# Mirko-Nava/BayesianNeuralNetworks

Measured on AMD Instinct MI355X. Metric: MC-samples/sec (node), 784-1200-1200-10 BayesianLinear MLP, batch 512, higher is better.
Workload: dtype bf16

## Files before the change

bayesianneuralnetworks_amd/_lib.py:

```python
import ctypes
import os

import torch

_HERE = os.path.dirname(os.path.abspath(__file__))
LIB_PATH = os.environ.get("BNN_HIP_LIB") or os.path.join(_HERE, "libbnn_hip.so")

F32, BF16, BF16X3 = 0, 1, 2
COMPUTE_F32, COMPUTE_BF16 = 0, 1
FLAG_RELU = 1
FLAG_X_BF16 = 2
E_ALIGN, E_UNSUPPORTED, E_DEVICE = -4, -6, -7
FLAG_Y_BF16 = 4


class BnnHipError(RuntimeError):
    pass


ABI_VERSION = 2


class Rng(ctypes.Structure):
    _fields_ = [("seed", ctypes.c_uint64),
# ... 39 lines not shown

_p = ctypes.c_void_p
_i64 = ctypes.c_int64
_int = ctypes.c_int
_f = ctypes.c_float
_rngp = ctypes.POINTER(Rng)

SIGNATURES = {
    "bnn_abi_version": (_int, []),
    "bnn_arch": (ctypes.c_char_p, []),
    "bnn_last_error": (ctypes.c_char_p, []),
    "bnn_launch_count": (ctypes.c_uint64, []),
    "bnn_set_workspace": (_int, [_int, _p, _i64]),
    "bnn_check_device": (_int, [_int, _p]),
    "bnn_sample_affine_eps": (_int, [_p, _p, _p, _p, _i64, _int, _p]),
    "bnn_sample_affine_philox": (_int, [_p, _p, _p, _i64, _int, _i64, _int, _rngp, _p]),
    "bnn_eps_philox": (_int, [_p, _i64, _int, _i64, _rngp, _p]),
    "bnn_sigma": (_int, [_p, _p, _i64, _p]),
    "bnn_sample_affine_bwd": (_int, [_p, _i64, _p, _p, _i64, _rngp, _i64, _int, _p, _p, _int, _p]),
    "bnn_rng_advance": (_int, [_p, ctypes.c_uint32, _p]),
    "bnn_prune_score": (_int, [_p, _p, _p, _i64, _p]),
    "bnn_kl_workspace_bytes": (_i64, [_int]),
    "bnn_kl_forward": (_int, [ctypes.POINTER(KlTensor), _int, _f, _p, _p, _p]),
    "bnn_kl_forward_partial": (_int, [ctypes.POINTER(KlTensor), _int, _p, _p]),
    "bnn_kl_backward": (_int, [ctypes.POINTER(KlTensor), _int, _f, _p, ctypes.POINTER(_p),
                               ctypes.POINTER(_p), _int, _p]),
    "bnn_linear_forward_sampled": (_int, [_p, _i64, _i64, _p, _p, _p, _p, _p, _i64, _i64, _i64, _i64,
                                          _i64, _int, _rngp, _rngp, _int, _int, _p]),
    "bnn_linear_forward_sampled_kl": (_int, [_p, _i64, _i64, _p, _p, _p, _p, _p, _i64, _i64, _i64, _i64,
                                             _i64, _int, _rngp, _rngp, _int, _int, ctypes.POINTER(KlTensor), _int, _p, _p]),
    "bnn_draw_multi": (_int, [ctypes.POINTER(DrawTensor), _int, _int, ctypes.POINTER(KlTensor), _int, _p, _p]),
    "bnn_dense_forward": (_int, [_p, _i64, _i64, _p, _i64, _i64, _p, _i64, _p, _i64, _i64, _i64, _i64, _i64, _int, _int, _p]),
    "bnn_dense_head_parts": (_int, [_i64, _i64, _int]),
    "bnn_dense_forward_head": (_int, [_p, _i64, _i64, _p, _i64, _i64, _p, _i64, _p, _i64, _i64, _p, _i64, _i64,
                                      _p, _i64, _i64, _i64, _int, _int, _p]),
    "bnn_dense_forward_x3_head": (_int, [_p, _i64, _i64, _i64, _p, _i64, _i64, _i64, _p, _i64, _p, _i64, _i64, _i64,
                                         _p, _i64, _i64, _p, _i64, _i64, _i64, _int, _int, _p]),
    "bnn_dense_forward_x3": (_int, [_p, _i64, _i64, _i64, _p, _i64, _i64, _i64, _p, _i64, _p, _i64, _i64, _i64,
                                    _i64, _i64, _i64, _int, _int, _p]),
    "bnn_split_bf16x3": (_int, [_p, _i64, _i64, _i64, _p, _i64, _i64, _p]),
    "bnn_transpose_bf16": (_int, [_p, _i64, _i64, _p, _i64, _i64, _i64, _i64, _int, _p]),
    "bnn_conv2d_dense_forward_x3": (_int, [_p, _i64, _p, _i64, _i64, _i64, _p, _i64, _p, _i64, ctypes.POINTER(Conv2dShape), _int, _int, _p]),
    "bnn_conv2d_dense_forward": (_int, [_p, _i64, _p, _i64, _i64, _p, _i64, _p, _i64, ctypes.POINTER(Conv2dShape), _int, _int, _p]),
    "bnn_conv2d_flipout_forward": (_int, [_p, _p, _i64, _p, _p, _p, ctypes.POINTER(Conv2dShape), _int, _p]),
    "bnn_conv2d_flipout_forward_x3": (_int, [_p, _p, _i64, _i64, _p, _p, _p, ctypes.POINTER(Conv2dShape), _int, _p]),
    "bnn_linear_forward": (_int, [_p, _i64, _i64, _p, _i64, _p, _i64, _p, _i64, _i64, _i64, _i64, _i64,
                                  _int, _int, _int, _p]),
    "bnn_linear_backward_input_sampled": (_int, [_p, _i64, _i64, _p, _p, _p, _i64, _i64, _i64, _i64, _i64, _int,
                                                 _rngp, _int, _int, _p]),
    "bnn_linear_backward_input": (_int, [_p, _i64, _i64, _p, _i64, _p, _i64, _i64, _i64, _i64, _i64, _int, _int, _p]),
    "bnn_linear_backward_weight_sampled": (_int, [_p, _i64, _i64, _p, _i64, _i64, _p, _p, _p, _p, _p, _p, _i64, _i64,
                                                  _i64, _int, _rngp, _rngp, ctypes.POINTER(KlFuse), _int, _int, _int, _p]),
    "bnn_linear_backward_narrow_sampled": (_int, [_p, _i64, _i64, _p, _i64, _i64, _p, _p, _p, _i64, _i64, _p, _p, _p, _p, _p,
                                                  _i64, _i64, _i64, _int, _rngp, _rngp, ctypes.POINTER(KlFuse), _int, _int, _p]),
    "bnn_linear_backward_weight": (_int, [_p, _i64, _i64, _p, _i64, _i64, _p, _i64, _i64, _i64, _i64, _int, _int,
                                          _int, _int, _p]),
    "bnn_colsum": (_int, [_p, _i64, _i64, _p, _i64, _i64, _int, _int, _p]),
    "bnn_relu_backward": (_int, [_p, _p, _p, _i64, _int, _p]),
    "bnn_adam_step": (_int, [ctypes.POINTER(AdamTensor), _int, _f, _f, _f, _f, _f, _p, _p]),
    "bnn_adam_step_advance": (_int, [ctypes.POINTER(AdamTensor), _int, _f, _f, _f, _f, _f, _p, _p, ctypes.c_uint32, _p]),
    "bnn_xent_workspace_bytes": (_i64, [_i64]),
    "bnn_softmax_xent": (_int, [_p, _p, _i64, _int, _p, _p, _p, _p]),
    "bnn_conv2d_im2col": (_int, [_p, _i64, ctypes.POINTER(Conv2dShape), _int, _p, _int, _p]),
    "bnn_conv2d_col2im": (_int, [_p, ctypes.POINTER(Conv2dShape), _int, _int, _p, _p]),
    "bnn_nchw_to_rows": (_int, [_p, _i64, _int, _int, _p, _int, _p]),
    "bnn_conv2d_workspace_bytes": (_i64, [ctypes.POINTER(Conv2dShape), _int, _int]),
# ... 117 lines not shown
```

bayesianneuralnetworks_amd/csrc/bnn_dense.hip:

```cpp
#include <cstdlib>
#include <type_traits>

#include "bnn_device.hpp"
#include "bnn_dma.hpp"
#include "bnn_kl_body.hpp"

namespace bnn {

typedef float f32x4 __attribute__((ext_vector_type(4)));
typedef __bf16 bf16x8 __attribute__((ext_vector_type(8)));

constexpr int kDrawMaxTensors = 8;
constexpr int kDrawSpreadBelow = 4096;

struct DrawTensorDev {
    const float *mu;
    const float *rho;
    void *out;
    int64_t out_sample_stride;
    int32_t rows, cols, ld;
    int32_t bf16;
    int32_t kind;
    int32_t perm_taps;
    int32_t first_item;
// ... 357 lines not shown
        }
    }
}

struct DenseParams {
    const uint16_t *A;
    int64_t a_sample_stride;
    int64_t lda;
    const uint16_t *W;
    int64_t w_sample_stride;
    int64_t ldw;
    const float *bias;
    int64_t bias_sample_stride;
    void *Y;
    int64_t y_sample_stride;
    int64_t ldy;
    int32_t M, N, K, S;
    int32_t ntm, ntn;
    int32_t flags;
    int32_t x3;
    int64_t a_plane_stride, w_plane_stride, y_plane_stride;
    const uint16_t *Wh;
    int64_t wh_sample_stride, ldwh;
    const float *bias_h;
    int64_t bias_h_sample_stride;
    float *P;
    int32_t Nh;
    int64_t wh_plane_stride;
};

constexpr int kDenseLoaderPrio = 1 << 21;
constexpr int kDenseNoXcdMap = 1 << 20;

__device__ __forceinline__ void dma_piece(const void *base, uint32_t voff, uint32_t lds)
{
    uint32_t keep;
    asm volatile("s_mov_b32 %0, m0\n\ts_mov_b32 m0, %3\n\ts_nop 0\n\tglobal_load_lds_dwordx4 %1, %2\n\ts_mov_b32 m0, %0"
                 : "=&s"(keep) : "v"(voff), "s"(base), "s"(lds) : "memory");
}

template <int TM, int TN, int NWM, int NWN, int ST, int YM, bool RELU, int DIAG = 0>
__global__ __launch_bounds__(512) void k_dense_bf16(const DenseParams p)
{
    constexpr int NWV = 4;
    constexpr bool INTERLEAVE = true;
    constexpr int MPR = DIAG == 3 ? 1 : DIAG == 4 ? 2 : TN >= 8 ? 2 : 1;
    static_assert(NWM * NWN == NWV, "four consumer waves");
    constexpr int WM = 16 * TM, WN = 16 * TN, BM = NWM * WM, BN = NWN * WN;
    constexpr int A_TOTAL = BM / 8;
    constexpr int B_TOTAL = BN / 8;
    static_assert(A_TOTAL % NWV == 0, "A pieces divide evenly over the loaders");
    constexpr int A_PIECES = A_TOTAL / NWV;
    constexpr int B_BASE = B_TOTAL / NWV, B_EXTRA = B_TOTAL % NWV;
    constexpr int A_STAGE = BM * 128;
    constexpr int B_STAGE = BN * 128;
    constexpr int STAGE = A_STAGE + B_STAGE;
    constexpr bool YBF = YM != 0;
    constexpr int ESZ = YBF ? 2 : 4;
    constexpr int EPI_BYTES = ST * STAGE / NWV;
    constexpr int EPI_A = (EPI_BYTES / (16 * (WN * ESZ + 16))) < TM ? (EPI_BYTES / (16 * (WN * ESZ + 16))) : TM;
    static_assert(EPI_A >= 1, "a quarter of the ring must hold at least 16 output rows (epilogue staging)");
    __shared__ __attribute__((aligned(16))) char lds[ST * STAGE];

    const int per_s = p.ntm * p.ntn;
    int s, t;
    {
        const int L = (int)blockIdx.x;
        if (p.flags & kDenseNoXcdMap) {
            s = L / per_s;
            t = L % per_s;
        } else if (p.S % 8 == 0) {
            const int idx = L >> 3;
            s = (L & 7) + 8 * (idx / per_s);
            t = idx % per_s;
        } else {
            const int total = per_s * p.S, x = L & 7;
            const int u = x * (total >> 3) + (x < (total & 7) ? x : (total & 7)) + (L >> 3);
            s = u / per_s;
            t = u % per_s;
        }
    }
    int mt, panel;
    if (per_s > 32 && !(p.flags & kDenseNoXcdMap)) {
        constexpr int GM = 4;
        const int grp = t / (GM * p.ntn), first = grp * GM;
        const int gm = p.ntm - first < GM ? p.ntm - first : GM;
        const int v = t - grp * (GM * p.ntn);
        mt = first + v % gm;
        panel = v / gm;
    } else {
        mt = t / p.ntn;
        panel = t % p.ntn;
    }
    const int m0 = mt * BM, n0 = panel * BN;
    const int tid = threadIdx.x, lane = tid & 63;
    const int wave = __builtin_amdgcn_readfirstlane(tid >> 6);
    const int nk = (p.K + 63) / 64 * (p.x3 ? 6 : 1);

    if (wave >= NWV) {
        const int lw = wave - NWV;
        if (p.flags & kDenseLoaderPrio) __builtin_amdgcn_s_setprio(2);
        const uint32_t ring = __builtin_amdgcn_readfirstlane(lds_addr_of(lds));
        const int prow = lane >> 3;
        const int schunk = (lane & 7) ^ prow;
        const char *a_base = reinterpret_cast<const char *>(p.A + (int64_t)s * p.a_sample_stride);
        const char *w_base = reinterpret_cast<const char *>(p.W + (int64_t)s * p.w_sample_stride);
        uint32_t a_off[A_PIECES], b_off[B_BASE + 1];
        uint32_t a_dst[A_PIECES], b_dst[B_BASE + 1];
#pragma unroll
        for (int j = 0; j < A_PIECES; ++j) {
            const int r0 = (lw + NWV * j) * 8;
            int m = m0 + r0 + prow;
            m = m < p.M ? m : p.M - 1;
            a_off[j] = (uint32_t)((int64_t)m * p.lda * 2);
            a_dst[j] = (uint32_t)((r0 / WM) * (ST * WM * 128) + (r0 % WM) * 128);
        }
#pragma unroll
        for (int j = 0; j < B_BASE + 1; ++j) {
            const int r0 = (lw + NWV * j) * 8;
            int n = n0 + r0 + prow;
            n = n < p.N ? n : p.N - 1;
            b_off[j] = (uint32_t)((int64_t)n * p.ldw * 2) + 16u * (uint32_t)schunk;
            b_dst[j] = (uint32_t)(ST * A_STAGE + (r0 / WN) * (ST * WN * 128) + (r0 % WN) * 128);
        }
        const uint32_t a_colmax = (uint32_t)(p.K * 2 - 16);
        auto run = [&](auto nbp_c) {
            constexpr int NBP = decltype(nbp_c)::value;
            constexpr int P = A_PIECES + NBP;
            auto issue = [&](int kt) {
                if constexpr (DIAG == 2 || DIAG == 5 || DIAG == 8 || DIAG == 9) return;
                const int stage = kt % ST;
                int kb = kt;
                const char *ab = a_base, *wb = w_base;
                if (p.x3) {
                    const int nkb = (p.K + 63) >> 6;
                    int pr = 5;
                    if (kt < 5 * nkb) { kb = kt / 5; pr = kt - 5 * kb; } else kb = kt - 5 * nkb;
                    ab += ((0x001102 >> (4 * pr)) & 3) * (p.a_plane_stride * 2);
                    wb += ((0x010120 >> (4 * pr)) & 3) * (p.w_plane_stride * 2);
                }
                const uint32_t colA0 = (uint32_t)(kb * 128 + 16 * schunk);
                const uint32_t colA = colA0 < a_colmax ? colA0 : a_colmax;
                const uint32_t colB = (uint32_t)(kb * 128);
                const uint32_t sa = ring + (uint32_t)(stage * (WM * 128)), sb = ring + (uint32_t)(stage * (WN * 128));
#pragma unroll
                for (int j = 0; j < A_PIECES; ++j)
                    dma_piece(ab, a_off[j] + colA, sa + a_dst[j]);
#pragma unroll
                for (int j = 0; j < NBP; ++j)
                    dma_piece(wb, b_off[j] + colB, sb + b_dst[j]);
            };
#pragma unroll
            for (int i = 0; i < ST - 1; ++i)
                if (i < nk) issue(i);
            for (int kt = 0; kt < nk; ++kt) {
                const int ahead = nk - 1 - kt < ST - 2 ? nk - 1 - kt : ST - 2;
                if (ST >= 4 && ahead == 2) asm volatile("s_waitcnt vmcnt(%0)" :: "n"(2 * P) : "memory");
                else if (ahead >= 1) asm volatile("s_waitcnt vmcnt(%0)" :: "n"(P) : "memory");
                else asm volatile("s_waitcnt vmcnt(0)" ::: "memory");
                if constexpr (DIAG != 5 && DIAG != 9) __builtin_amdgcn_s_barrier();
                if (kt + ST - 1 < nk) issue(kt + ST - 1);
            }
            __builtin_amdgcn_s_barrier();
        };
        if (lw < B_EXTRA) run(std::integral_constant<int, B_BASE + 1>{});
        else run(std::integral_constant<int, B_BASE>{});
        return;
    }

    static_assert(ST == 3 || ST == 4, "ring depth");
    uint64_t stamp[5] = {0, 0, 0, 0, 0};
    if constexpr (DIAG >= 6) stamp[0] = __builtin_amdgcn_s_memrealtime();
    const int fi = lane & 15, fq = lane >> 4;
    const int wm = wave / NWN, wn = wave % NWN;
    const char *a_rows = lds + wm * (ST * WM * 128);
    const char *b_rows = lds + ST * A_STAGE + wn * (ST * WN * 128);
    __builtin_amdgcn_s_setprio(1);
    f32x4 acc[TM][TN];
#pragma unroll
    for (int a = 0; a < TM; ++a)
#pragma unroll
        for (int b = 0; b < TN; ++b) acc[a][b] = f32x4{0.f, 0.f, 0.f, 0.f};
    const int fbase0 = fi * 128 + (((0 + fq) ^ (fi & 7)) << 4);
    const int fbase1 = fi * 128 + (((4 + fq) ^ (fi & 7)) << 4);
    uint4 fa[2][TM], fb[2][TN];
    auto rd = [&](auto buf_c, uint32_t stage, auto h_c) {
        constexpr int buf = decltype(buf_c)::value, h = decltype(h_c)::value;
        if constexpr (DIAG == 1 || DIAG == 7) return;
        const char *As = a_rows + (stage * (uint32_t)(WM * 128) + (uint32_t)(h ? fbase1 : fbase0));
        const char *Bs = b_rows + (stage * (uint32_t)(WN * 128) + (uint32_t)(h ? fbase1 : fbase0));
#pragma unroll
        for (int b = 0; b < TN; ++b) fb[buf][b] = *reinterpret_cast<const uint4 *>(Bs + b * 2048);
#pragma unroll
        for (int a = 0; a < TM; ++a) fa[buf][a] = *reinterpret_cast<const uint4 *>(As + a * 2048);
    };
    auto mm = [&](auto buf_c) {
        constexpr int buf = decltype(buf_c)::value;
        if constexpr (DIAG == 1 || DIAG == 7) return;
#pragma unroll
        for (int a = 0; a < TM; ++a)
#pragma unroll
            for (int b = 0; b < TN; ++b)
                acc[a][b] = __builtin_amdgcn_mfma_f32_16x16x32_bf16(__builtin_bit_cast(bf16x8, fb[buf][b]),
                                                                    __builtin_bit_cast(bf16x8, fa[buf][a]), acc[a][b], 0, 0, 0);
    };
    using I0 = std::integral_constant<int, 0>;
    using I1 = std::integral_constant<int, 1>;
    auto interleave = [&]() {
        if constexpr ((DIAG == 0 || (DIAG >= 3 && DIAG != 7)) && INTERLEAVE) {
            constexpr int NI = (TM * TN) / MPR < TM + TN ? (TM * TN) / MPR : TM + TN;
#pragma unroll
            for (int i = 0; i < NI; ++i) {
                __builtin_amdgcn_sched_group_barrier(0x008, MPR, 0);
                __builtin_amdgcn_sched_group_barrier(0x100, 1, 0);
            }
            if constexpr (TM + TN > NI) __builtin_amdgcn_sched_group_barrier(0x100, TM + TN - NI, 0);
            if constexpr (TM * TN > MPR * NI) __builtin_amdgcn_sched_group_barrier(0x008, TM * TN - MPR * NI, 0);
        }
    };
    auto first_half = [&](uint32_t stage) {
        rd(I1{}, stage, I1{});
        if constexpr (!INTERLEAVE) __builtin_amdgcn_sched_barrier(0);
        mm(I0{});
        interleave();
        __builtin_amdgcn_sched_barrier(0);
    };
    auto second_half = [&](uint32_t next) {
        asm volatile("s_waitcnt lgkmcnt(0)" ::: "memory");
        if constexpr (DIAG != 5 && DIAG != 9) __builtin_amdgcn_s_barrier();
        asm volatile("" ::: "memory");
        rd(I0{}, next, I0{});
        if constexpr (!INTERLEAVE) __builtin_amdgcn_sched_barrier(0);
        mm(I1{});
        interleave();
        __builtin_amdgcn_sched_barrier(0);
    };
    const float *bias = p.bias ? p.bias + (int64_t)s * p.bias_sample_stride : nullptr;
    const int mw = m0 + wm * WM, nw = n0 + wn * WN;
    constexpr bool BIAS_PRE = TM * TN <= 20;
    float bv[TN][4];
    auto load_bias = [&]() {
#pragma unroll
        for (int b = 0; b < TN; ++b)
#pragma unroll
            for (int r = 0; r < 4; ++r) {
                const int n = nw + b * 16 + fq * 4 + r;
                bv[b][r] = (bias && n < p.N) ? bias[n] : 0.f;
            }
    };
    if constexpr (BIAS_PRE) load_bias();
    if (DIAG == 0 && (nw >= p.N || mw >= p.M)) {
        for (int kt = 0; kt < nk + 1; ++kt) __builtin_amdgcn_s_barrier();
        if constexpr (YM == 3) {
            float *P = p.P + ((int64_t)(panel * NWN + wn) * p.S + s) * (int64_t)p.M * p.Nh;
            for (int i = lane; i < WM * p.Nh; i += 64) {
                const int m = mw + i / p.Nh;
                if (m < p.M) P[(int64_t)m * p.Nh + (i % p.Nh)] = 0.f;
            }
        }
        return;
    }
    if constexpr (DIAG != 5 && DIAG != 9) __builtin_amdgcn_s_barrier();
    asm volatile("" ::: "memory");
    if constexpr (DIAG >= 6) stamp[1] = __builtin_amdgcn_s_memrealtime();
    rd(I0{}, 0u, I0{});
    uint32_t stage = 0;
    for (int kt = 0; kt + 1 < nk; ++kt) {
        const uint32_t next = stage + 1 == (uint32_t)ST ? 0u : stage + 1;
        first_half(stage);
        second_half(next);
        stage = next;
    }
    first_half(stage);
    mm(I1{});
    __builtin_amdgcn_sched_barrier(0);
    __builtin_amdgcn_s_setprio(0);
    asm volatile("s_waitcnt lgkmcnt(0)" ::: "memory");
    __builtin_amdgcn_s_barrier();
    asm volatile("" ::: "memory");
    if constexpr (DIAG >= 6) stamp[2] = __builtin_amdgcn_s_memrealtime();
    auto leave_stamps = [&]() {
        if constexpr (DIAG >= 6) {
            stamp[3] = __builtin_amdgcn_s_memrealtime();
            asm volatile("s_waitcnt vmcnt(0)" ::: "memory");
            stamp[4] = __builtin_amdgcn_s_memrealtime();
            if (wave == 0 && lane == 0 && p.P) {
                uint64_t *q = reinterpret_cast<uint64_t *>(p.P) + (int64_t)blockIdx.x * 5;
                for (int i = 0; i < 5; ++i) q[i] = stamp[i];
            }
        }
    };

    if constexpr (!BIAS_PRE) load_bias();
    const int64_t ybase = (int64_t)s * p.y_sample_stride * ESZ;
    auto vals = [&](int a, int b, float (&v)[4]) {
#pragma unroll
        for (int r = 0; r < 4; ++r) {
            v[r] = acc[a][b][r] + bv[b][r];
            if (RELU) v[r] = fmaxf(v[r], 0.f);
        }
    };
    if constexpr (YM == 3) {
        constexpr bool X3_HEAD_FITS = 3 * WM * (WN * 2 + 16) <= EPI_BYTES;
        if constexpr (X3_HEAD_FITS) if (p.x3) {
            constexpr int pitch = WN * 2 + 16;
            char *T = lds + wave * EPI_BYTES;
#pragma unroll
            for (int a = 0; a < TM; ++a)
#pragma unroll
                for (int b = 0; b < TN; ++b) {
                    float v[4];
                    vals(a, b, v);
                    uint32_t h0, m0, l0, h1, m1, l1;
                    split_bf16x3(v[0], v[1], h0, m0, l0);
                    split_bf16x3(v[2], v[3], h1, m1, l1);
                    char *q = T + (a * 16 + fi) * pitch + (b * 16 + fq * 4) * 2;
                    *reinterpret_cast<uint2 *>(q) = make_uint2(h0, h1);
                    *reinterpret_cast<uint2 *>(q + WM * pitch) = make_uint2(m0, m1);
                    *reinterpret_cast<uint2 *>(q + 2 * WM * pitch) = make_uint2(l0, l1);
                }
            __builtin_amdgcn_fence(__ATOMIC_RELEASE, "workgroup");
            __builtin_amdgcn_wave_barrier();
            const int Nh = p.Nh;
            const int hrow = fi < Nh ? fi : Nh - 1;
            const uint16_t *wh = p.Wh + (int64_t)s * p.wh_sample_stride + (int64_t)hrow * p.ldwh;
            f32x4 hacc[TM], hsm[TM];
#pragma unroll
            for (int a = 0; a < TM; ++a) { hacc[a] = f32x4{0.f, 0.f, 0.f, 0.f}; hsm[a] = hacc[a]; }
            constexpr int NC = (WN + 31) / 32;
#pragma unroll
            for (int c = 0; c < NC; ++c) {
                const int kcol = 32 * c + 8 * fq;
                const int n = nw + kcol;
                const bool okb = kcol < WN && fi < Nh && n + 8 <= (int)p.ldwh;
                uint4 bf[3];
#pragma unroll
                for (int pl = 0; pl < 3; ++pl)
                    bf[pl] = okb ? *reinterpret_cast<const uint4 *>(wh + pl * p.wh_plane_stride + n) : make_uint4(0u, 0u, 0u, 0u);
#pragma unroll
                for (int a = 0; a < TM; ++a) {
                    uint4 af[3];
#pragma unroll
                    for (int pl = 0; pl < 3; ++pl)
                        af[pl] = kcol < WN ? *reinterpret_cast<const uint4 *>(T + pl * WM * pitch + (a * 16 + fi) * pitch + kcol * 2) : make_uint4(0u, 0u, 0u, 0u);
                    auto mf = [&](f32x4 c4, int pa, int pw) {
                        return __builtin_amdgcn_mfma_f32_16x16x32_bf16(__builtin_bit_cast(bf16x8, af[pa]), __builtin_bit_cast(bf16x8, bf[pw]), c4, 0, 0, 0);
                    };
                    hsm[a] = mf(mf(mf(mf(mf(hsm[a], 2, 0), 0, 2), 1, 1), 1, 0), 0, 1);
                    hacc[a] = mf(hacc[a], 0, 0);
                }
            }
            const int part = panel * NWN + wn;
            float hb = 0.f;
            if (part == 0 && p.bias_h && fi < Nh) hb = p.bias_h[(int64_t)s * p.bias_h_sample_stride + fi];
            float *P = p.P + ((int64_t)part * p.S + s) * (int64_t)p.M * Nh;
#pragma unroll
            for (int a = 0; a < TM; ++a)
#pragma unroll
                for (int r = 0; r < 4; ++r) {
                    const int m = mw + a * 16 + fq * 4 + r;
                    if (m < p.M && fi < Nh) P[(int64_t)m * Nh + fi] = (hacc[a][r] + hsm[a][r]) + hb;
                }
            return;
        }
        constexpr int pitch = WN * 2 + 16;
        static_assert(WM * pitch <= EPI_BYTES, "the wave's quarter of the ring holds its bf16 tile");
        char *T = lds + wave * EPI_BYTES;
#pragma unroll
        for (int a = 0; a < TM; ++a)
#pragma unroll
            for (int b = 0; b < TN; ++b) {
                float v[4];
                vals(a, b, v);
                *reinterpret_cast<uint2 *>(T + (a * 16 + fi) * pitch + (b * 16 + fq * 4) * 2) = make_uint2(pack_bf16x2(v[0], v[1]), pack_bf16x2(v[2], v[3]));
            }
        __builtin_amdgcn_fence(__ATOMIC_RELEASE, "workgroup");
        __builtin_amdgcn_wave_barrier();
        const int Nh = p.Nh;
        const int hrow = fi < Nh ? fi : Nh - 1;
        const uint16_t *wh = p.Wh + (int64_t)s * p.wh_sample_stride + (int64_t)hrow * p.ldwh;
        f32x4 hacc[TM];
#pragma unroll
        for (int a = 0; a < TM; ++a) hacc[a] = f32x4{0.f, 0.f, 0.f, 0.f};
        constexpr int NC = (WN + 31) / 32;
#pragma unroll
        for (int c = 0; c < NC; ++c) {
            const int kcol = 32 * c + 8 * fq;
            const int n = nw + kcol;
            uint4 bf = make_uint4(0u, 0u, 0u, 0u);
            if (kcol < WN && fi < Nh && n + 8 <= (int)p.ldwh) bf = *reinterpret_cast<const uint4 *>(wh + n);
#pragma unroll
            for (int a = 0; a < TM; ++a) {
                uint4 af = make_uint4(0u, 0u, 0u, 0u);
                if (kcol < WN) af = *reinterpret_cast<const uint4 *>(T + (a * 16 + fi) * pitch + kcol * 2);
                hacc[a] = __builtin_amdgcn_mfma_f32_16x16x32_bf16(__builtin_bit_cast(bf16x8, af), __builtin_bit_cast(bf16x8, bf), hacc[a], 0, 0, 0);
            }
        }
        const int part = panel * NWN + wn;
        float hb = 0.f;
        if (part == 0 && p.bias_h && fi < Nh) hb = p.bias_h[(int64_t)s * p.bias_h_sample_stride + fi];
        float *P = p.P + ((int64_t)part * p.S + s) * (int64_t)p.M * Nh;
#pragma unroll
        for (int a = 0; a < TM; ++a)
#pragma unroll
            for (int r = 0; r < 4; ++r) {
                const int m = mw + a * 16 + fq * 4 + r;
                if (m < p.M && fi < Nh) P[(int64_t)m * Nh + fi] = hacc[a][r] + hb;
            }
        return;
    }
    auto plane_of = [&](float v, int pl) -> uint16_t {
        const uint16_t h = f2bf(v);
        if (pl == 0) return h;
        const float r = v - __uint_as_float((uint32_t)h << 16);
        const uint16_t m = f2bf(r);
        if (pl == 1) return m;
        return f2bf(r - __uint_as_float((uint32_t)m << 16));
    };
    constexpr int NP = YM == 2 ? 3 : 1;
    const bool wide = nw + WN <= p.N && mw + WM <= p.M && (p.ldy * ESZ) % 16 == 0 && (nw * ESZ) % 16 == 0 &&
                      ((reinterpret_cast<uintptr_t>(p.Y) + ybase) & 15u) == 0 && (NP == 1 || (p.y_plane_stride * ESZ) % 16 == 0);
    if (wide) {
        char *T = lds + wave * EPI_BYTES;
        constexpr int row_bytes = WN * ESZ;
        constexpr int pitch = row_bytes + 16;
        constexpr int cpr = row_bytes / 16;
#pragma unroll
        for (int pl = 0; pl < NP; ++pl) {
            char *Y8 = reinterpret_cast<char *>(p.Y) + ybase + ((int64_t)pl * p.y_plane_stride + (int64_t)mw * p.ldy + nw) * ESZ;
#pragma unroll
            for (int a0 = 0; a0 < TM; a0 += EPI_A) {
#pragma unroll
                for (int b = 0; b < TN; ++b)
#pragma unroll
                    for (int a = a0; a < a0 + EPI_A && a < TM; ++a) {
                        float v[4];
                        vals(a, b, v);
                        char *q = T + ((a - a0) * 16 + fi) * pitch + (b * 16 + fq * 4) * ESZ;
                        if (YM == 2)
                            *reinterpret_cast<uint2 *>(q) = make_uint2((uint32_t)plane_of(v[0], pl) | ((uint32_t)plane_of(v[1], pl) << 16),
                                                                       (uint32_t)plane_of(v[2], pl) | ((uint32_t)plane_of(v[3], pl) << 16));
                        else if (YM == 1) *reinterpret_cast<uint2 *>(q) = make_uint2(pack_bf16x2(v[0], v[1]), pack_bf16x2(v[2], v[3]));
                        else *reinterpret_cast<float4 *>(q) = make_float4(v[0], v[1], v[2], v[3]);
                    }
                __builtin_amdgcn_fence(__ATOMIC_RELEASE, "workgroup");
                __builtin_amdgcn_wave_barrier();
                const int nrows = (TM - a0 < EPI_A ? TM - a0 : EPI_A) * 16;
                for (int c = lane; c < nrows * cpr; c += 64) {
                    const int row = c / cpr, cc = c - row * cpr;
                    *reinterpret_cast<uint4 *>(Y8 + (int64_t)(a0 * 16 + row) * p.ldy * ESZ + cc * 16) =
                        *reinterpret_cast<const uint4 *>(T + row * pitch + cc * 16);
                }
                __builtin_amdgcn_fence(__ATOMIC_RELEASE, "workgroup");
                __builtin_amdgcn_wave_barrier();
            }
        }
        leave_stamps();
        return;
    }
    float *Yf = reinterpret_cast<float *>(p.Y) + (int64_t)s * p.y_sample_stride;
    uint16_t *Yh = reinterpret_cast<uint16_t *>(p.Y) + (int64_t)s * p.y_sample_stride;
#pragma unroll
    for (int a = 0; a < TM; ++a) {
        const int m = mw + a * 16 + fi;
        if (m >= p.M) continue;
#pragma unroll
        for (int b = 0; b < TN; ++b) {
            float v[4];
            vals(a, b, v);
#pragma unroll
            for (int r = 0; r < 4; ++r) {
                const int n = nw + b * 16 + fq * 4 + r;
                if (n >= p.N) continue;
                if (YM == 2) {
#pragma unroll
                    for (int pl = 0; pl < 3; ++pl) Yh[(int64_t)pl * p.y_plane_stride + (int64_t)m * p.ldy + n] = plane_of(v[r], pl);
                } else if (YM == 1) Yh[(int64_t)m * p.ldy + n] = f2bf(v[r]);
                else Yf[(int64_t)m * p.ldy + n] = v[r];
            }
        }
    }
}

constexpr int kHeadMaxSteps = 16;

__global__ __launch_bounds__(256) void k_head_bf16(const DenseParams p)
{
    __shared__ float red[4][16][17];
    const int ntm = p.ntm;
    const int s = (int)blockIdx.x / ntm, mt = (int)blockIdx.x % ntm;
    const int tid = threadIdx.x, lane = tid & 63, wave = tid >> 6;
    const int fi = lane & 15, fq = lane >> 4;
    const int nk = (p.K + 31) / 32;
    const int per = (nk + 3) / 4;
    const int k0 = wave * per, k1 = (k0 + per < nk) ? k0 + per : nk;
    int m = mt * 16 + fi;
    m = m < p.M ? m : p.M - 1;
    int n = fi < p.N ? fi : p.N - 1;
    const uint16_t *arow = p.A + (int64_t)s * p.a_sample_stride + (int64_t)m * p.lda;
    const uint16_t *wrow = p.W + (int64_t)s * p.w_sample_stride + (int64_t)n * p.ldw;
    uint4 af[kHeadMaxSteps], bfr[kHeadMaxSteps];
    const int kmax = p.K - 8;
    f32x4 acc = f32x4{0.f, 0.f, 0.f, 0.f};
    const int npass = p.x3 ? 6 : 1;
    for (int pass = 0; pass < npass; ++pass) {
        const uint16_t *ar = arow, *wr = wrow;
        if (p.x3) {
            ar += ((0x001102 >> (4 * pass)) & 3) * p.a_plane_stride;
            wr += ((0x010120 >> (4 * pass)) & 3) * p.w_plane_stride;
        }
#pragma unroll
        for (int i = 0; i < kHeadMaxSteps; ++i) {
            const int kt = k0 + i;
            int ka = kt * 32 + 8 * fq;
// ... 591 lines not shown
                    d.kl_prior_mu = kl_tensors[j].prior_mu; d.kl_prior_sigma = kl_tensors[j].prior_sigma;
                    in_items = true;
                }
            }
            L.kl.pg_first[j] = launched;
            if (!in_items) launched += nb;
        }
        L.kl.pg_first[kl_ntensors] = launched;
        L.kl.nblocks = launched;
        grid += L.kl.nblocks;
    }
    int split = 1;
    while (split < nsamples && (int64_t)L.draw_blocks * split < 1024) split *= 2;
    if (split > nsamples) split = nsamples;
    static const int force_split = [] { const char *e = getenv("BNN_DRAW_SPLIT"); return e ? atoi(e) : 0; }();
    if (force_split >= 1 && force_split <= nsamples) split = force_split;
    static const int unroll = [] { const char *e = getenv("BNN_DRAW_UNROLL"); return e ? atoi(e) : 1; }();
    if (unroll == 2) hipLaunchKernelGGL(k_draw_multi<2>, dim3((unsigned)grid, (unsigned)split), dim3(256), 0, (hipStream_t)stream, L);
    else if (unroll == 4) hipLaunchKernelGGL(k_draw_multi<4>, dim3((unsigned)grid, (unsigned)split), dim3(256), 0, (hipStream_t)stream, L);
    else if (unroll == 8) hipLaunchKernelGGL(k_draw_multi<8>, dim3((unsigned)grid, (unsigned)split), dim3(256), 0, (hipStream_t)stream, L);
    else
    hipLaunchKernelGGL(k_draw_multi<1>, dim3((unsigned)grid, (unsigned)split), dim3(256), 0, (hipStream_t)stream, L);
    return check_launch(who);
}

int bnn_dense_forward(const void *x, int64_t x_sample_stride, int64_t ldx,
                      const void *w, int64_t w_sample_stride, int64_t ldw,
                      const float *b, int64_t b_sample_stride,
                      void *y, int64_t y_sample_stride, int64_t ldy,
                      int64_t M, int64_t N, int64_t K, int nsamples, int flags, void *stream)
{
    return dense_launch("bnn_dense_forward", x, 0, x_sample_stride, ldx, w, 0, w_sample_stride, ldw, b, b_sample_stride,
                        y, 0, y_sample_stride, ldy, M, N, K, nsamples, flags, false, stream);
}

int bnn_dense_head_parts(int64_t M, int64_t N, int nsamples)
{
    if (M < 1 || N < 17 || nsamples < 1) return 0;
    const int tile = dense_pick_tile(M, N, nsamples);
    const int bn = tile == 0 ? 80 : tile == 2 ? 128 : 160;
    const int nwn = (tile == 0 || tile == 2) ? 1 : 2;
    return (int)((N + bn - 1) / bn) * nwn;
}

int bnn_dense_forward_head(const void *x, int64_t x_sample_stride, int64_t ldx,
                           const void *w, int64_t w_sample_stride, int64_t ldw,
                           const float *b, int64_t b_sample_stride,
                           const void *w_head, int64_t wh_sample_stride, int64_t ldwh,
                           const float *b_head, int64_t bh_sample_stride, int64_t n_head,
                           float *partials, int64_t M, int64_t N, int64_t K, int nsamples, int flags, void *stream)
{
    HeadArgs h{w_head, 0, wh_sample_stride, ldwh, b_head, bh_sample_stride, partials, n_head};
    return dense_launch("bnn_dense_forward_head", x, 0, x_sample_stride, ldx, w, 0, w_sample_stride, ldw, b, b_sample_stride,
                        nullptr, 0, 0, N, M, N, K, nsamples, flags | BNN_FLAG_Y_BF16, false, stream, &h);
}

int bnn_dense_forward_x3_head(const void *x, int64_t x_plane_stride, int64_t x_sample_stride, int64_t ldx,
                              const void *w, int64_t w_plane_stride, int64_t w_sample_stride, int64_t ldw,
                              const float *b, int64_t b_sample_stride,
                              const void *w_head, int64_t wh_plane_stride, int64_t wh_sample_stride, int64_t ldwh,
                              const float *b_head, int64_t bh_sample_stride, int64_t n_head,
                              float *partials, int64_t M, int64_t N, int64_t K, int nsamples, int flags, void *stream)
{
    if (wh_plane_stride <= 0) { set_error("bnn_dense_forward_x3_head: plane stride of the head's weights"); return BNN_E_SHAPE; }
    HeadArgs h{w_head, wh_plane_stride, wh_sample_stride, ldwh, b_head, bh_sample_stride, partials, n_head};
    return dense_launch("bnn_dense_forward_x3_head", x, x_plane_stride, x_sample_stride, ldx, w, w_plane_stride, w_sample_stride, ldw,
// ... 155 lines not shown
```

include/bnn_hip.h:

```cpp
#ifndef BNN_HIP_H
#define BNN_HIP_H

#include <stdint.h>

#ifdef __cplusplus
extern "C" {
#endif

#define BNN_ABI_VERSION 2

enum {
    BNN_OK = 0,
    BNN_E_NULL = -1,
    BNN_E_SHAPE = -2,
    BNN_E_DTYPE = -3,
    BNN_E_ALIGN = -4,
    BNN_E_RANGE = -5,
    BNN_E_UNSUPPORTED = -6,
    BNN_E_DEVICE = -7
};

enum { BNN_F32 = 0, BNN_BF16 = 1,
       BNN_BF16X3 = 2  };

// ... 63 lines not shown
int bnn_linear_forward_sampled(const void *x, int64_t x_sample_stride, int64_t ldx,
                               const float *mu_w, const float *rho_w,
                               const float *mu_b, const float *rho_b,
                               void *y, int64_t y_sample_stride, int64_t ldy,
                               int64_t M, int64_t N, int64_t K, int nsamples,
                               const bnn_rng_t *rng_w, const bnn_rng_t *rng_b,
                               int compute, int flags, void *stream);
int bnn_linear_forward_sampled_kl(const void *x, int64_t x_sample_stride, int64_t ldx,
                                  const float *mu_w, const float *rho_w, const float *mu_b,
                                  const float *rho_b, void *y, int64_t y_sample_stride, int64_t ldy,
                                  int64_t M, int64_t N, int64_t K, int nsamples, const bnn_rng_t *rng_w,
                                  const bnn_rng_t *rng_b, int compute, int flags,
                                  const bnn_kl_tensor_t *tensors, int ntensors, void *kl_workspace, void *stream);
typedef struct bnn_draw_tensor {
    const float *mu;
    const float *rho;
    int64_t rows, cols;
    void *out;
    int64_t ld;
    int64_t out_sample_stride;
    int out_dtype;
    int kind;
    int taps;
    bnn_rng_t rng;
} bnn_draw_tensor_t;
int bnn_draw_multi(const bnn_draw_tensor_t *tensors, int ntensors, int nsamples,
                   const bnn_kl_tensor_t *kl_tensors, int kl_ntensors, void *kl_workspace, void *stream);
int bnn_dense_forward(const void *x, int64_t x_sample_stride, int64_t ldx,
                      const void *w, int64_t w_sample_stride, int64_t ldw,
                      const float *b, int64_t b_sample_stride,
                      void *y, int64_t y_sample_stride, int64_t ldy,
                      int64_t M, int64_t N, int64_t K, int nsamples, int flags, void *stream);
int bnn_dense_head_parts(int64_t M, int64_t N, int nsamples);
int bnn_dense_forward_head(const void *x, int64_t x_sample_stride, int64_t ldx,
                           const void *w, int64_t w_sample_stride, int64_t ldw,
                           const float *b, int64_t b_sample_stride,
                           const void *w_head, int64_t wh_sample_stride, int64_t ldwh,
                           const float *b_head, int64_t bh_sample_stride, int64_t n_head,
                           float *partials, int64_t M, int64_t N, int64_t K, int nsamples, int flags, void *stream);
int bnn_dense_forward_x3_head(const void *x, int64_t x_plane_stride, int64_t x_sample_stride, int64_t ldx,
                              const void *w, int64_t w_plane_stride, int64_t w_sample_stride, int64_t ldw,
                              const float *b, int64_t b_sample_stride,
                              const void *w_head, int64_t wh_plane_stride, int64_t wh_sample_stride, int64_t ldwh,
                              const float *b_head, int64_t bh_sample_stride, int64_t n_head,
                              float *partials, int64_t M, int64_t N, int64_t K, int nsamples, int flags, void *stream);
int bnn_dense_forward_x3(const void *x, int64_t x_plane_stride, int64_t x_sample_stride, int64_t ldx,
                         const void *w, int64_t w_plane_stride, int64_t w_sample_stride, int64_t ldw,
                         const float *b, int64_t b_sample_stride,
                         void *y, int64_t y_plane_stride, int64_t y_sample_stride, int64_t ldy,
                         int64_t M, int64_t N, int64_t K, int nsamples, int flags, void *stream);
int bnn_split_bf16x3(const float *x, int64_t rows, int64_t cols, int64_t ldx, void *out, int64_t ld_out, int64_t plane_stride,
                     void *stream);
int bnn_transpose_bf16(const void *in, int64_t in_batch_stride, int64_t ld_in, void *out, int64_t out_batch_stride, int64_t ld_out,
                       int64_t rows, int64_t cols, int batch, void *stream);

int bnn_linear_forward(const float *x, int64_t x_sample_stride, int64_t ldx,
                       const float *w, int64_t w_sample_stride,
                       const float *b, int64_t b_sample_stride,
                       float *y, int64_t y_sample_stride, int64_t ldy,
                       int64_t M, int64_t N, int64_t K, int nsamples,
                       int compute, int flags, void *stream);

int bnn_linear_backward_input_sampled(const void *gy, int64_t gy_sample_stride, int64_t ldgy,
                                      const float *mu_w, const float *rho_w,
                                      void *gx, int64_t gx_sample_stride, int64_t ldgx,
                                      int64_t M, int64_t N, int64_t K, int nsamples,
// ... 119 lines not shown
```

Before: 188,700.

## Trim dense GEMM tail-tile work and stage bias through LDS via DMA

Loader waves now compute how many B rows the tile actually covers and issue only those DMA pieces. For single-column-wave TN=8 tiles, the consumer picks a reduced TNE at runtime so partial last N tiles skip their MFMAs and LDS reads. Bias for large tiles is prefetched into an extra LDS slot by a loader wave instead of being read from global memory in the epilogue, and base pointers are forced into SGPRs. This adds template instantiations and code size, and the wide-store path now masks partial columns. A query function for the chosen tile is also exported.

```diff
diff --git a/bayesianneuralnetworks_amd/_lib.py b/bayesianneuralnetworks_amd/_lib.py
--- a/bayesianneuralnetworks_amd/_lib.py
+++ b/bayesianneuralnetworks_amd/_lib.py
@@ -95,6 +95,7 @@
     "bnn_draw_multi": (_int, [ctypes.POINTER(DrawTensor), _int, _int, ctypes.POINTER(KlTensor), _int, _p, _p]),
     "bnn_dense_forward": (_int, [_p, _i64, _i64, _p, _i64, _i64, _p, _i64, _p, _i64, _i64, _i64, _i64, _i64, _int, _int, _p]),
     "bnn_dense_head_parts": (_int, [_i64, _i64, _int]),
+    "bnn_dense_tile": (_int, [_i64, _i64, _int]),
     "bnn_dense_forward_head": (_int, [_p, _i64, _i64, _p, _i64, _i64, _p, _i64, _p, _i64, _i64, _p, _i64, _i64,
                                       _p, _i64, _i64, _i64, _int, _int, _p]),
     "bnn_dense_forward_x3_head": (_int, [_p, _i64, _i64, _i64, _p, _i64, _i64, _i64, _p, _i64, _p, _i64, _i64, _i64,
diff --git a/bayesianneuralnetworks_amd/csrc/bnn_dense.hip b/bayesianneuralnetworks_amd/csrc/bnn_dense.hip
--- a/bayesianneuralnetworks_amd/csrc/bnn_dense.hip
+++ b/bayesianneuralnetworks_amd/csrc/bnn_dense.hip
@@ -413,6 +413,13 @@
 constexpr int kDenseLoaderPrio = 1 << 21;
 constexpr int kDenseNoXcdMap = 1 << 20;
 
+__device__ __forceinline__ const char *sgpr_ptr(const void *p)
+{
+    const uint64_t v = reinterpret_cast<uint64_t>(p);
+    const uint32_t lo = __builtin_amdgcn_readfirstlane((uint32_t)v), hi = __builtin_amdgcn_readfirstlane((uint32_t)(v >> 32));
+    return reinterpret_cast<const char *>(((uint64_t)hi << 32) | lo);
+}
+
 __device__ __forceinline__ void dma_piece(const void *base, uint32_t voff, uint32_t lds)
 {
     uint32_t keep;
@@ -420,12 +427,26 @@
                  : "=&s"(keep) : "v"(voff), "s"(base), "s"(lds) : "memory");
 }
 
+__device__ __forceinline__ void dma_dword(const void *base, uint32_t voff, uint32_t lds)
+{
+    uint32_t keep;
+    asm volatile("s_mov_b32 %0, m0\n\ts_mov_b32 m0, %3\n\ts_nop 0\n\tglobal_load_lds_dword %1, %2\n\ts_mov_b32 m0, %0"
+                 : "=&s"(keep) : "v"(voff), "s"(base), "s"(lds) : "memory");
+}
+
+template <int LO, int HI, class F>
+__device__ __forceinline__ void with_count(int n, F &&f)
+{
+    if constexpr (LO >= HI) f(std::integral_constant<int, HI>{});
+    else if (n <= LO) f(std::integral_constant<int, LO>{});
+    else with_count<LO + 1, HI>(n, f);
+}
+
 template <int TM, int TN, int NWM, int NWN, int ST, int YM, bool RELU, int DIAG = 0>
 __global__ __launch_bounds__(512) void k_dense_bf16(const DenseParams p)
 {
     constexpr int NWV = 4;
     constexpr bool INTERLEAVE = true;
-    constexpr int MPR = DIAG == 3 ? 1 : DIAG == 4 ? 2 : TN >= 8 ? 2 : 1;
     static_assert(NWM * NWN == NWV, "four consumer waves");
     constexpr int WM = 16 * TM, WN = 16 * TN, BM = NWM * WM, BN = NWN * WN;
     constexpr int A_TOTAL = BM / 8;
@@ -441,7 +462,11 @@
     constexpr int EPI_BYTES = ST * STAGE / NWV;
     constexpr int EPI_A = (EPI_BYTES / (16 * (WN * ESZ + 16))) < TM ? (EPI_BYTES / (16 * (WN * ESZ + 16))) : TM;
     static_assert(EPI_A >= 1, "a quarter of the ring must hold at least 16 output rows (epilogue staging)");
-    __shared__ __attribute__((aligned(16))) char lds[ST * STAGE];
+    constexpr bool BIAS_PRE = TM * TN <= 20;
+    constexpr int BIAS_SLOT = BIAS_PRE ? 0 : BN * 4;
+    static_assert(BN % 64 == 0 || BIAS_PRE, "the bias slot is filled 64 columns at a time");
+    __shared__ __attribute__((aligned(16))) char lds[ST * STAGE + BIAS_SLOT];
+    constexpr bool TN_SPLIT = NWN == 1 && TN == 8 && (DIAG == 0 || DIAG == 6);
 
     const int per_s = p.ntm * p.ntn;
     int s, t;
@@ -477,6 +502,8 @@
     const int tid = threadIdx.x, lane = tid & 63;
     const int wave = __builtin_amdgcn_readfirstlane(tid >> 6);
     const int nk = (p.K + 63) / 64 * (p.x3 ? 6 : 1);
+    const int pcols = p.N - n0;
+    const int brows = TN_SPLIT ? (pcols < BN ? (pcols + 15) / 16 * 16 : BN) : (pcols < BN ? (pcols + WN - 1) / WN * WN : BN);
 
     if (wave >= NWV) {
         const int lw = wave - NWV;
@@ -484,8 +511,8 @@
         const uint32_t ring = __builtin_amdgcn_readfirstlane(lds_addr_of(lds));
         const int prow = lane >> 3;
         const int schunk = (lane & 7) ^ prow;
-        const char *a_base = reinterpret_cast<const char *>(p.A + (int64_t)s * p.a_sample_stride);
-        const char *w_base = reinterpret_cast<const char *>(p.W + (int64_t)s * p.w_sample_stride);
+        const char *a_base = sgpr_ptr(p.A + (int64_t)s * p.a_sample_stride);
+        const char *w_base = sgpr_ptr(p.W + (int64_t)s * p.w_sample_stride);
         uint32_t a_off[A_PIECES], b_off[B_BASE + 1];
         uint32_t a_dst[A_PIECES], b_dst[B_BASE + 1];
 #pragma unroll
@@ -505,7 +532,17 @@
             b_dst[j] = (uint32_t)(ST * A_STAGE + (r0 / WN) * (ST * WN * 128) + (r0 % WN) * 128);
         }
         const uint32_t a_colmax = (uint32_t)(p.K * 2 - 16);
-        auto run = [&](auto nbp_c) {
+        if constexpr (!BIAS_PRE) {
+            if (lw == 0 && p.bias) {
+                const char *bb = sgpr_ptr(p.bias + (int64_t)s * p.bias_sample_stride);
+#pragma unroll
+                for (int j = 0; j < BN / 64; ++j) {
+                    const int n = n0 + 64 * j + lane;
+                    dma_dword(bb, (uint32_t)(n < p.N ? n : p.N - 1) * 4u, ring + (uint32_t)(ST * STAGE + 256 * j));
+                }
+            }
+        }
+        auto run = [&](auto nbp_c) __attribute__((always_inline)) {
             constexpr int NBP = decltype(nbp_c)::value;
             constexpr int P = A_PIECES + NBP;
             auto issue = [&](int kt) {
@@ -544,8 +581,24 @@
             }
             __builtin_amdgcn_s_barrier();
         };
-        if (lw < B_EXTRA) run(std::integral_constant<int, B_BASE + 1>{});
-        else run(std::integral_constant<int, B_BASE>{});
+        const int nbp_all = lw < B_EXTRA ? B_BASE + 1 : B_BASE;
+        const int nbp_read = (brows / 8 - lw + NWV - 1) / NWV;
+        const int nbp = __builtin_amdgcn_readfirstlane(nbp_read < nbp_all ? nbp_read : nbp_all);
+        if (nbp == B_BASE + 1) run(std::integral_constant<int, B_BASE + 1>{});
+        else if (nbp == B_BASE) run(std::integral_constant<int, B_BASE>{});
+        else if constexpr (B_BASE >= 1) {
+            if (nbp == B_BASE - 1) run(std::integral_constant<int, B_BASE - 1>{});
+            else if constexpr (B_BASE >= 2) {
+                if (nbp == B_BASE - 2) run(std::integral_constant<int, B_BASE - 2>{});
+                else if constexpr (B_BASE >= 3) {
+                    if (nbp == B_BASE - 3) run(std::integral_constant<int, B_BASE - 3>{});
+                    else if constexpr (B_BASE >= 4) {
+                        if (nbp == B_BASE - 4) run(std::integral_constant<int, B_BASE - 4>{});
+                        else if constexpr (B_BASE >= 5) { if (nbp == B_BASE - 5) run(std::integral_constant<int, B_BASE - 5>{}); }
+                    }
+                }
+            }
+        }
         return;
     }
 
@@ -557,21 +610,24 @@
     const char *a_rows = lds + wm * (ST * WM * 128);
     const char *b_rows = lds + ST * A_STAGE + wn * (ST * WN * 128);
     __builtin_amdgcn_s_setprio(1);
-    f32x4 acc[TM][TN];
+    auto consume = [&](auto tne_c) __attribute__((always_inline)) {
+    constexpr int TNE = decltype(tne_c)::value, WNE = 16 * TNE;
+    constexpr int MPRE = DIAG == 3 ? 1 : DIAG == 4 ? 2 : TNE >= 8 ? 2 : 1;
+    f32x4 acc[TM][TNE];
 #pragma unroll
     for (int a = 0; a < TM; ++a)
 #pragma unroll
-        for (int b = 0; b < TN; ++b) acc[a][b] = f32x4{0.f, 0.f, 0.f, 0.f};
+        for (int b = 0; b < TNE; ++b) acc[a][b] = f32x4{0.f, 0.f, 0.f, 0.f};
     const int fbase0 = fi * 128 + (((0 + fq) ^ (fi & 7)) << 4);
     const int fbase1 = fi * 128 + (((4 + fq) ^ (fi & 7)) << 4);
-    uint4 fa[2][TM], fb[2][TN];
+    uint4 fa[2][TM], fb[2][TNE];
     auto rd = [&](auto buf_c, uint32_t stage, auto h_c) {
         constexpr int buf = decltype(buf_c)::value, h = decltype(h_c)::value;
         if constexpr (DIAG == 1 || DIAG == 7) return;
         const char *As = a_rows + (stage * (uint32_t)(WM * 128) + (uint32_t)(h ? fbase1 : fbase0));
         const char *Bs = b_rows + (stage * (uint32_t)(WN * 128) + (uint32_t)(h ? fbase1 : fbase0));
 #pragma unroll
-        for (int b = 0; b < TN; ++b) fb[buf][b] = *reinterpret_cast<const uint4 *>(Bs + b * 2048);
+        for (int b = 0; b < TNE; ++b) fb[buf][b] = *reinterpret_cast<const uint4 *>(Bs + b * 2048);
 #pragma unroll
         for (int a = 0; a < TM; ++a) fa[buf][a] = *reinterpret_cast<const uint4 *>(As + a * 2048);
     };
@@ -581,7 +637,7 @@
 #pragma unroll
         for (int a = 0; a < TM; ++a)
 #pragma unroll
-            for (int b = 0; b < TN; ++b)
+            for (int b = 0; b < TNE; ++b)
                 acc[a][b] = __builtin_amdgcn_mfma_f32_16x16x32_bf16(__builtin_bit_cast(bf16x8, fb[buf][b]),
                                                                     __builtin_bit_cast(bf16x8, fa[buf][a]), acc[a][b], 0, 0, 0);
     };
@@ -589,14 +645,14 @@
     using I1 = std::integral_constant<int, 1>;
     auto interleave = [&]() {
         if constexpr ((DIAG == 0 || (DIAG >= 3 && DIAG != 7)) && INTERLEAVE) {
-            constexpr int NI = (TM * TN) / MPR < TM + TN ? (TM * TN) / MPR : TM + TN;
+            constexpr int NI = (TM * TNE) / MPRE < TM + TNE ? (TM * TNE) / MPRE : TM + TNE;
 #pragma unroll
             for (int i = 0; i < NI; ++i) {
-                __builtin_amdgcn_sched_group_barrier(0x008, MPR, 0);
+                __builtin_amdgcn_sched_group_barrier(0x008, MPRE, 0);
                 __builtin_amdgcn_sched_group_barrier(0x100, 1, 0);
             }
-            if constexpr (TM + TN > NI) __builtin_amdgcn_sched_group_barrier(0x100, TM + TN - NI, 0);
-            if constexpr (TM * TN > MPR * NI) __builtin_amdgcn_sched_group_barrier(0x008, TM * TN - MPR * NI, 0);
+            if constexpr (TM + TNE > NI) __builtin_amdgcn_sched_group_barrier(0x100, TM + TNE - NI, 0);
+            if constexpr (TM * TNE > MPRE * NI) __builtin_amdgcn_sched_group_barrier(0x008, TM * TNE - MPRE * NI, 0);
         }
     };
     auto first_half = [&](uint32_t stage) {
@@ -618,16 +674,22 @@
     };
     const float *bias = p.bias ? p.bias + (int64_t)s * p.bias_sample_stride : nullptr;
     const int mw = m0 + wm * WM, nw = n0 + wn * WN;
-    constexpr bool BIAS_PRE = TM * TN <= 20;
-    float bv[TN][4];
+    float bv[TNE][4];
     auto load_bias = [&]() {
 #pragma unroll
-        for (int b = 0; b < TN; ++b)
+        for (int b = 0; b < TNE; ++b) {
+            float4 v4 = make_float4(0.f, 0.f, 0.f, 0.f);
+            if constexpr (!BIAS_PRE) {
+                if (bias) v4 = *reinterpret_cast<const float4 *>(lds + ST * STAGE + (wn * WN + b * 16 + fq * 4) * 4);
+            }
+            const float vv[4] = {v4.x, v4.y, v4.z, v4.w};
 #pragma unroll
             for (int r = 0; r < 4; ++r) {
                 const int n = nw + b * 16 + fq * 4 + r;
-                bv[b][r] = (bias && n < p.N) ? bias[n] : 0.f;
-            }
+                if constexpr (BIAS_PRE) bv[b][r] = (bias && n < p.N) ? bias[n] : 0.f;
+                else bv[b][r] = n < p.N ? vv[r] : 0.f;
+            }
+        }
     };
     if constexpr (BIAS_PRE) load_bias();
     if (DIAG == 0 && (nw >= p.N || mw >= p.M)) {
@@ -689,7 +751,7 @@
 #pragma unroll
             for (int a = 0; a < TM; ++a)
 #pragma unroll
-                for (int b = 0; b < TN; ++b) {
+                for (int b = 0; b < TNE; ++b) {
                     float v[4];
                     vals(a, b, v);
                     uint32_t h0, m0, l0, h1, m1, l1;
@@ -708,12 +770,12 @@
             f32x4 hacc[TM], hsm[TM];
 #pragma unroll
             for (int a = 0; a < TM; ++a) { hacc[a] = f32x4{0.f, 0.f, 0.f, 0.f}; hsm[a] = hacc[a]; }
-            constexpr int NC = (WN + 31) / 32;
+            constexpr int NC = (WNE + 31) / 32;
 #pragma unroll
             for (int c = 0; c < NC; ++c) {
                 const int kcol = 32 * c + 8 * fq;
                 const int n = nw + kcol;
-                const bool okb = kcol < WN && fi < Nh && n + 8 <= (int)p.ldwh;
+                const bool okb = kcol < WNE && fi < Nh && n + 8 <= (int)p.ldwh;
                 uint4 bf[3];
 #pragma unroll
                 for (int pl = 0; pl < 3; ++pl)
@@ -723,7 +785,7 @@
                     uint4 af[3];
 #pragma unroll
                     for (int pl = 0; pl < 3; ++pl)
-                        af[pl] = kcol < WN ? *reinterpret_cast<const uint4 *>(T + pl * WM * pitch + (a * 16 + fi) * pitch + kcol * 2) : make_uint4(0u, 0u, 0u, 0u);
+                        af[pl] = kcol < WNE ? *reinterpret_cast<const uint4 *>(T + pl * WM * pitch + (a * 16 + fi) * pitch + kcol * 2) : make_uint4(0u, 0u, 0u, 0u);
                     auto mf = [&](f32x4 c4, int pa, int pw) {
                         return __builtin_amdgcn_mfma_f32_16x16x32_bf16(__builtin_bit_cast(bf16x8, af[pa]), __builtin_bit_cast(bf16x8, bf[pw]), c4, 0, 0, 0);
                     };
@@ -750,7 +812,7 @@
 #pragma unroll
         for (int a = 0; a < TM; ++a)
 #pragma unroll
-            for (int b = 0; b < TN; ++b) {
+            for (int b = 0; b < TNE; ++b) {
                 float v[4];
                 vals(a, b, v);
                 *reinterpret_cast<uint2 *>(T + (a * 16 + fi) * pitch + (b * 16 + fq * 4) * 2) = make_uint2(pack_bf16x2(v[0], v[1]), pack_bf16x2(v[2], v[3]));
@@ -763,17 +825,17 @@
         f32x4 hacc[TM];
 #pragma unroll
         for (int a = 0; a < TM; ++a) hacc[a] = f32x4{0.f, 0.f, 0.f, 0.f};
-        constexpr int NC = (WN + 31) / 32;
+        constexpr int NC = (WNE + 31) / 32;
 #pragma unroll
         for (int c = 0; c < NC; ++c) {
             const int kcol = 32 * c + 8 * fq;
             const int n = nw + kcol;
             uint4 bf = make_uint4(0u, 0u, 0u, 0u);
-            if (kcol < WN && fi < Nh && n + 8 <= (int)p.ldwh) bf = *reinterpret_cast<const uint4 *>(wh + n);
+            if (kcol < WNE && fi < Nh && n + 8 <= (int)p.ldwh) bf = *reinterpret_cast<const uint4 *>(wh + n);
 #pragma unroll
             for (int a = 0; a < TM; ++a) {
                 uint4 af = make_uint4(0u, 0u, 0u, 0u);
-                if (kcol < WN) af = *reinterpret_cast<const uint4 *>(T + (a * 16 + fi) * pitch + kcol * 2);
+                if (kcol < WNE) af = *reinterpret_cast<const uint4 *>(T + (a * 16 + fi) * pitch + kcol * 2);
                 hacc[a] = __builtin_amdgcn_mfma_f32_16x16x32_bf16(__builtin_bit_cast(bf16x8, af), __builtin_bit_cast(bf16x8, bf), hacc[a], 0, 0, 0);
             }
         }
@@ -799,20 +861,22 @@
         return f2bf(r - __uint_as_float((uint32_t)m << 16));
     };
     constexpr int NP = YM == 2 ? 3 : 1;
-    const bool wide = nw + WN <= p.N && mw + WM <= p.M && (p.ldy * ESZ) % 16 == 0 && (nw * ESZ) % 16 == 0 &&
+    const int vcols = p.N - nw < WNE ? p.N - nw : WNE;
+    const bool wide = (vcols * ESZ) % 16 == 0 && mw + WM <= p.M && (p.ldy * ESZ) % 16 == 0 && (nw * ESZ) % 16 == 0 &&
                       ((reinterpret_cast<uintptr_t>(p.Y) + ybase) & 15u) == 0 && (NP == 1 || (p.y_plane_stride * ESZ) % 16 == 0);
     if (wide) {
         char *T = lds + wave * EPI_BYTES;
         constexpr int row_bytes = WN * ESZ;
         constexpr int pitch = row_bytes + 16;
-        constexpr int cpr = row_bytes / 16;
+        constexpr int cpr = WNE * ESZ / 16;
+        const int vcpr = vcols * ESZ / 16;
 #pragma unroll
         for (int pl = 0; pl < NP; ++pl) {
             char *Y8 = reinterpret_cast<char *>(p.Y) + ybase + ((int64_t)pl * p.y_plane_stride + (int64_t)mw * p.ldy + nw) * ESZ;
 #pragma unroll
             for (int a0 = 0; a0 < TM; a0 += EPI_A) {
 #pragma unroll
-                for (int b = 0; b < TN; ++b)
+                for (int b = 0; b < TNE; ++b)
 #pragma unroll
                     for (int a = a0; a < a0 + EPI_A && a < TM; ++a) {
                         float v[4];
@@ -829,6 +893,7 @@
                 const int nrows = (TM - a0 < EPI_A ? TM - a0 : EPI_A) * 16;
                 for (int c = lane; c < nrows * cpr; c += 64) {
                     const int row = c / cpr, cc = c - row * cpr;
+                    if (cc < vcpr)
                     *reinterpret_cast<uint4 *>(Y8 + (int64_t)(a0 * 16 + row) * p.ldy * ESZ + cc * 16) =
                         *reinterpret_cast<const uint4 *>(T + row * pitch + cc * 16);
                 }
@@ -846,7 +911,7 @@
         const int m = mw + a * 16 + fi;
         if (m >= p.M) continue;
 #pragma unroll
-        for (int b = 0; b < TN; ++b) {
+        for (int b = 0; b < TNE; ++b) {
             float v[4];
             vals(a, b, v);
 #pragma unroll
@@ -861,6 +926,10 @@
             }
         }
     }
+    leave_stamps();
+    };
+    if constexpr (TN_SPLIT) with_count<1, TN>(brows / 16, consume);
+    else consume(std::integral_constant<int, TN>{});
 }
 
 constexpr int kHeadMaxSteps = 16;
@@ -1518,6 +1587,13 @@
 {
     return dense_launch("bnn_dense_forward", x, 0, x_sample_stride, ldx, w, 0, w_sample_stride, ldw, b, b_sample_stride,
                         y, 0, y_sample_stride, ldy, M, N, K, nsamples, flags, false, stream);
+}
+
+int bnn_dense_tile(int64_t M, int64_t N, int nsamples)
+{
+    if (M < 1 || N < 1 || nsamples < 1) return -1;
+    if (N <= 16) return 5;
+    return dense_pick_tile(M, N, nsamples);
 }
 
 int bnn_dense_head_parts(int64_t M, int64_t N, int nsamples)
diff --git a/include/bnn_hip.h b/include/bnn_hip.h
--- a/include/bnn_hip.h
+++ b/include/bnn_hip.h
@@ -119,6 +119,7 @@
                       void *y, int64_t y_sample_stride, int64_t ldy,
                       int64_t M, int64_t N, int64_t K, int nsamples, int flags, void *stream);
 int bnn_dense_head_parts(int64_t M, int64_t N, int nsamples);
+int bnn_dense_tile(int64_t M, int64_t N, int nsamples);
 int bnn_dense_forward_head(const void *x, int64_t x_sample_stride, int64_t ldx,
                            const void *w, int64_t w_sample_stride, int64_t ldw,
                            const float *b, int64_t b_sample_stride,
```

Result: no change. 188,300 (median of 6 runs) (-0.2%).
